# dalek-cryptography/curve25519-dalek

Measured on NVIDIA H100. Metric: Pippenger MSM points/sec, higher is better.
Workload: dtype exact integers: f64 limbs (radix 2^51, FP64 pipe) in the bucket kernel, u32 limbs (radix 2^25.5) elsewhere

## Files before the change

### curve25519_dalek_b200/csrc/engine.h

```cpp
#pragma once
#include <cuda_runtime.h>
#include <stddef.h>
#include <stdint.h>
#include <cstdio>
#include <string>
#include <utility>
#include <vector>

#include "../../include/dalek_b200.h"
#include "ge.cuh"

struct DevBuf {
    void *p = nullptr;
    size_t cap = 0;
};

struct dalek_b200_ctx {
    int device = 0;
    int sm_count = 132;
    cudaStream_t stream = nullptr;
    cudaStream_t stream2 = nullptr;
    cudaStream_t stream_copy = nullptr;
    cudaStream_t stream3 = nullptr;
    cudaStream_t stream_hash = nullptr;
    cudaEvent_t ev_hram[8] = {};
    cudaEvent_t ev_a = nullptr, ev_b = nullptr, ev_fork = nullptr, ev_join = nullptr, ev_join2 = nullptr;
    cudaEvent_t ev_call0 = nullptr, ev_call1 = nullptr;
    cudaEvent_t ev_prep[8][2] = {};
    int prep_pieces = 0;
    float last_prep_ms = 0.f;
    cudaEvent_t ev_grp[8] = {nullptr, nullptr, nullptr, nullptr, nullptr, nullptr, nullptr, nullptr};
    std::string last_error;
    uint64_t launches = 0;
    long opt_window_bits = 0;
    long opt_verify_chunk = 0;
    long opt_host_chunks = 8;
    long opt_trace = 0;
    long opt_precomp_tables = 0;
    long opt_double_base_comb = 1;
    long opt_dedupe_keys = 1;
    long opt_verify_pieces = 4;
    long opt_decompress_f64 = 1;
    long opt_acc_tma = 0;
    long opt_transcript_warp = 1;
    long opt_transcript_blocks = 1;
    long opt_each_comb = 1;
    long opt_small_straus = 1;
    long opt_field_f64 = 1;
    float last_kernel_ms = 0.f;
    float last_call_ms = 0.f;
    int last_kernel_launches = 0;
    bool async_open = false;
    DevBuf scalars, points_in, points, digits, counts, offsets, sorted, buckets, red_a, red_b, red_c,
        red_d, key_pts, result, flags, misc0, misc1, misc2, misc3, misc4, misc5, zs, base_table, ntasks, task_off, tasks, task_sums, msg_offs, sum_desc, sum_part, key_table, key_acc, task_order, sig_status, misc6, each_pow, each_tab, each_kstat;
    DevBuf prep_prod;
    uint32_t hash_seed[4] = {0x243F6A88u, 0x85A308D3u, 0x13198A2Eu, 0x03707344u};
    int sum_desc_c = -1;
    bool base_table_ready = false;
    bool each_attr_set = false;
    bool comb_attr_set = false;
    DevBuf comb_base_table;
    bool comb_base_table_ready = false;
    void *h_pinned = nullptr;
    size_t h_pinned_cap = 0;
    size_t last_zs_n = 0;
    std::vector<std::pair<const char *, cudaEvent_t>> trace;
};

#define CUDA_TRY(ctx, expr)                                                                      \
    do {                                                                                         \
        cudaError_t _e = (expr);                                                                 \
        if (_e != cudaSuccess) {                                                                 \
            (ctx)->last_error = std::string(#expr) + ": " + cudaGetErrorString(_e);              \
            return -3;                                                                           \
        }                                                                                        \
    } while (0)

inline float elapsed_ms(cudaEvent_t a, cudaEvent_t b)
{
    float ms = 0.f;
    if (cudaEventElapsedTime(&ms, a, b) == cudaSuccess) return ms;
    cudaGetLastError();
    return -1.f;
}

struct CallTimer {
    dalek_b200_ctx *ctx;
    explicit CallTimer(dalek_b200_ctx *c) : ctx(c) { if (ctx) cudaEventRecord(ctx->ev_call0, ctx->stream); }
    ~CallTimer()
    {
        if (!ctx) return;
        float ms = 0.f;
        if (cudaEventRecord(ctx->ev_call1, ctx->stream) == cudaSuccess && cudaEventSynchronize(ctx->ev_call1) == cudaSuccess &&
            (ms = elapsed_ms(ctx->ev_call0, ctx->ev_call1)) >= 0.f)
            ctx->last_call_ms = ms;
    }
};

inline void trace_mark(dalek_b200_ctx *ctx, const char *name, cudaStream_t st)
{
    if (!ctx->opt_trace) return;
    cudaEvent_t e;
    if (cudaEventCreate(&e) != cudaSuccess) return;
    cudaEventRecord(e, st);
    ctx->trace.push_back({name, e});
}
inline void trace_dump(dalek_b200_ctx *ctx)
{
    if (!ctx->opt_trace) return;
    cudaDeviceSynchronize();
// ... 66 lines not shown
```

### curve25519_dalek_b200/csrc/msm.cu

```cuda
#include <algorithm>
#include <cstdio>
#include <utility>
#include <vector>

#include "../../include/dalek_b200.h"
#include "engine.h"
#include "ge64.cuh"
#include "warp4.cuh"
#include "warp4_f64.cuh"

static inline unsigned cdiv(size_t a, unsigned b) { return (unsigned)((a + b - 1) / b); }

int ws_reserve(dalek_b200_ctx *ctx, DevBuf &b, size_t bytes)
{
    if (bytes <= b.cap) return 0;
    if (b.p) { cudaFree(b.p); b.p = nullptr; b.cap = 0; }
    size_t want = bytes + bytes / 8 + 256;
    cudaError_t e = cudaMalloc(&b.p, want);
    if (e != cudaSuccess) { ctx->last_error = std::string("cudaMalloc: ") + cudaGetErrorString(e); return DALEK_E_NOMEM; }
    b.cap = want;
    return 0;
}

int pinned_reserve(dalek_b200_ctx *ctx, size_t bytes)
{
    if (bytes <= ctx->h_pinned_cap) return 0;
    if (ctx->h_pinned) cudaFreeHost(ctx->h_pinned);
    ctx->h_pinned = nullptr; ctx->h_pinned_cap = 0;
    cudaError_t e = cudaMallocHost(&ctx->h_pinned, bytes + 4096);
    if (e != cudaSuccess) { ctx->last_error = std::string("cudaMallocHost: ") + cudaGetErrorString(e); return DALEK_E_NOMEM; }
    ctx->h_pinned_cap = bytes + 4096;
    return 0;
}

template <int F64>
__global__ void __launch_bounds__(128, 3) k_prep_compressed(const uint4 *__restrict__ in, ge_niels_packed *__restrict__ out, size_t n,
                                  int *__restrict__ bad)
{
    size_t i = (size_t)blockIdx.x * blockDim.x + threadIdx.x;
    if (i >= n) return;
    uint4 a = in[2 * i], b = in[2 * i + 1];
    uint32_t s[8] = {a.x, a.y, a.z, a.w, b.x, b.y, b.z, b.w};
    fe x, y;
    uint32_t ok = ge_decompress_affine<F64>(x, y, s);
    if (!ok) { atomicOr(bad, 1); fe_0(x); fe_1(y); }
    ge_niels nl; ge_affine_to_niels(nl, x, y);
    ge_niels_packed p; ge_niels_pack(p, nl);
    uint4 *o = reinterpret_cast<uint4 *>(out + i);
#pragma unroll
    for (int k = 0; k < 6; k++) o[k] = make_uint4(p.w[4 * k], p.w[4 * k + 1], p.w[4 * k + 2], p.w[4 * k + 3]);
}

template <int F64>
__global__ void k_prep_ristretto(const uint32_t *__restrict__ in, ge_niels_packed *__restrict__ out, size_t n, int *__restrict__ bad)
{
    size_t i = (size_t)blockIdx.x * blockDim.x + threadIdx.x;
    if (i >= n) return;
    uint32_t enc[8];
#pragma unroll
    for (int k = 0; k < 8; k++) enc[k] = in[8 * i + k];
    ge_p3 P;
// ... 756 lines not shown
                }
            }
        };
        if (len) prefetch(e_next, 0);
        if (!TMA) asm volatile("cp.async.commit_group;" ::: "memory");
        for (uint32_t k = 0; k < len; k++) {
            const uint32_t e = e_next, neg = e >> 31;
            const int buf = k & 1;
            if (k + 1 < len) { e_next = idx[k + 1]; prefetch(e_next, buf ^ 1); }
            uint32_t words[NQ * 4];
            if (TMA) {
                const uint32_t bar = (uint32_t)__cvta_generic_to_shared(&s_bar[buf][threadIdx.x]);
                const uint32_t parity = (k >> 1) & 1u;
                uint32_t done;
                do {
                    asm volatile("{ .reg .pred p; mbarrier.try_wait.parity.shared::cta.b64 p, [%1], %2; selp.u32 %0, 1, 0, p; }"
                                 : "=r"(done) : "r"(bar), "r"(parity) : "memory");
                } while (!done);
                const uint4 *sp = reinterpret_cast<const uint4 *>(&s_bulk[buf][threadIdx.x][0]);
#pragma unroll
                for (int q = 0; q < NQ; q++) { uint4 v = sp[q]; words[4 * q] = v.x; words[4 * q + 1] = v.y; words[4 * q + 2] = v.z; words[4 * q + 3] = v.w; }
            } else {
                asm volatile("cp.async.commit_group;" ::: "memory");
                asm volatile("cp.async.wait_group 1;" ::: "memory");
#pragma unroll
                for (int q = 0; q < NQ; q++) { uint4 v = s_pts[buf][q][threadIdx.x]; words[4 * q] = v.x; words[4 * q + 1] = v.y; words[4 * q + 2] = v.z; words[4 * q + 3] = v.w; }
            }
            ge_niels_packed pk;
#pragma unroll
            for (int q = 0; q < 24; q++) pk.w[q] = words[q];
            ge64_niels nl; ge64_niels_unpack(nl, pk);
            ge64_madd(acc64, acc64, nl, neg);
        }
        ge64_to_p3(acc, acc64);
    } else {
    if (fold_old) load_p3(acc, buckets + t); else ge_p3_identity(acc);
    for (uint32_t k = 0; k < len; k++) {
        uint32_t e = idx[k];
        uint32_t neg = e >> 31, pi = e & 0x7fffffffu;
        const uint4 *src = reinterpret_cast<const uint4 *>(reinterpret_cast<const ge_niels_packed *>(points) + pi);
        ge_niels_packed pk;
#pragma unroll
        for (int q = 0; q < 6; q++) { uint4 v = __ldg(src + q); pk.w[4 * q] = v.x; pk.w[4 * q + 1] = v.y; pk.w[4 * q + 2] = v.z; pk.w[4 * q + 3] = v.w; }
        ge_niels nl; ge_niels_unpack(nl, pk);
        ge_madd(acc, acc, nl, neg);
    }
    }
    ge_p3_raw r; ge_p3_store_raw(r, acc);
    uint4 *o = reinterpret_cast<uint4 *>(!split ? buckets + t : task_sums + p);
#pragma unroll
    for (int q = 0; q < 10; q++) o[q] = make_uint4(r.w[4 * q], r.w[4 * q + 1], r.w[4 * q + 2], r.w[4 * q + 3]);
}


__global__ void __launch_bounds__(128)
k_heavy_fixup(const uint32_t *__restrict__ heavy, const uint32_t *__restrict__ ntasks, const uint32_t *__restrict__ task_off,
              const uint32_t *__restrict__ win_base, uint32_t nbuckets, uint32_t w0, uint32_t w1,
              const ge_p3_raw *__restrict__ task_sums, ge_p3_raw *__restrict__ buckets, int first)
{
    const uint32_t lane = threadIdx.x & 31, role = lane & 3, grp = lane >> 2;
    const uint32_t nwarps = (gridDim.x * blockDim.x) >> 5;
    const uint32_t nheavy = heavy[0];
    for (uint32_t h = (blockIdx.x * blockDim.x + threadIdx.x) >> 5; h < nheavy; h += nwarps) {
        uint32_t tb = heavy[1 + h];
        if (tb / nbuckets < w0 || tb / nbuckets >= w1) continue;
        uint32_t kk = ntasks[tb];
        uint32_t base = win_base[tb / nbuckets] + task_off[tb];
        w4_point acc, x;
        if (first || grp != 0) w4_identity(acc); else w4_load(acc, buckets + tb);
        for (uint32_t j0 = 0; j0 < kk; j0 += 8) {
            uint32_t j = j0 + grp;
            if (j < kk) w4_load(x, task_sums + base + j); else w4_identity(x);
            w4_add(acc, x, role);
        }
        for (int d = 16; d >= 4; d >>= 1) { w4_shfl_down(x, acc, d); w4_add(acc, x, role); }
        if (grp == 0) w4_store(buckets + tb, acc, role);
    }
}

__device__ __forceinline__ void load_p3_f64(ge64_p3 &o, const ge_p3_raw *src)
{
    ge_p3 q; load_p3(q, src);
    fe64_from_fe_limbs(o.X, q.X); fe64_from_fe_limbs(o.Y, q.Y); fe64_from_fe_limbs(o.Z, q.Z); fe64_from_fe_limbs(o.T, q.T);
}

__global__ void __launch_bounds__(32)
k_chunk_reduce_f64(const ge_p3_raw *__restrict__ S_in, uint32_t n_in, uint32_t m, uint32_t n_out, uint32_t nwin,
                   ge_p3_raw *__restrict__ S_out, ge_p3_raw *__restrict__ W_out)
{
    const uint32_t t = blockIdx.x * blockDim.x + threadIdx.x;
    if (t >= n_out * nwin) return;
    const uint32_t w = t / n_out, q = t % n_out;
    const ge_p3_raw *S = S_in + (size_t)w * n_in + (size_t)q * m;
    fe64 d2; fe64_const_2d(d2);
    ge64_p3 run, acc, x;
    load_p3_f64(run, S + (m - 1));
    acc = run;
    ge_p3 nxt;
    if (m > 1) load_p3(nxt, S + (m - 2));
#pragma unroll 1
    for (uint32_t r = m - 1; r-- > 0;) {
        fe64_from_fe_limbs(x.X, nxt.X); fe64_from_fe_limbs(x.Y, nxt.Y); fe64_from_fe_limbs(x.Z, nxt.Z); fe64_from_fe_limbs(x.T, nxt.T);
        if (r > 0) load_p3(nxt, S + (r - 1));
        ge64_add_p3(run, run, x, d2);
        ge64_add_p3(acc, acc, run, d2);
    }
    ge_p3 o; ge_p3_raw raw;
    ge64_to_p3(o, run); ge_p3_store_raw(raw, o);
    uint4 *d = reinterpret_cast<uint4 *>(S_out + t);
#pragma unroll
    for (int k = 0; k < 10; k++) d[k] = make_uint4(raw.w[4 * k], raw.w[4 * k + 1], raw.w[4 * k + 2], raw.w[4 * k + 3]);
    ge64_to_p3(o, acc); ge_p3_store_raw(raw, o);
    d = reinterpret_cast<uint4 *>(W_out + t);
#pragma unroll
    for (int k = 0; k < 10; k++) d[k] = make_uint4(raw.w[4 * k], raw.w[4 * k + 1], raw.w[4 * k + 2], raw.w[4 * k + 3]);
}

__global__ void __launch_bounds__(128)
k_chunk_reduce(const ge_p3_raw *__restrict__ S_in, uint32_t n_in, uint32_t m, uint32_t one_based, uint32_t n_out,
               uint32_t nwin, ge_p3_raw *__restrict__ S_out, ge_p3_raw *__restrict__ W_out)
{
    const uint32_t role = threadIdx.x & 3;
    const uint32_t total = n_out * nwin;
    uint32_t t = (blockIdx.x * blockDim.x + threadIdx.x) >> 2;
    if (((blockIdx.x * blockDim.x + (threadIdx.x & ~31u)) >> 2) >= total) return;
    const bool live = t < total;
    if (!live) t = total - 1;
    const uint32_t w = t / n_out, q = t % n_out;
    const ge_p3_raw *S = S_in + (size_t)w * n_in + (size_t)q * m;
    w4_point run, acc, x;
    w4_load(run, S + (m - 1));
    acc = run;
    for (uint32_t r = m - 1; r-- > 1;) {
        w4_load(x, S + r);
        w4_add(run, x, role);
        w4_add(acc, run, role);
    }
    if (m > 1) {
        w4_load(x, S);
        w4_add(run, x, role);
        if (one_based) w4_add(acc, run, role);
    } else if (!one_based) {
        w4_identity(acc);
    }
    if (live) { w4_store(S_out + t, run, role); w4_store(W_out + t, acc, role); }
}

#define SUM_PIECE 256u
__global__ void __launch_bounds__(128)
k_plain_sum(const ge_p3_raw *__restrict__ pool, const uint2 *__restrict__ desc, ge_p3_raw *__restrict__ out)
{
    __shared__ ge_p3_raw sh[32];
    const uint32_t role = threadIdx.x & 3, grp = threadIdx.x >> 2;
    const uint2 d = desc[blockIdx.x];
    const ge_p3_raw *a = pool + d.x;
    const uint32_t len = d.y;
    w4_point acc, x;
    w4_identity(acc);
    for (uint32_t i0 = 0; i0 < len; i0 += 32) {
        uint32_t i = i0 + grp;
        if (i < len) w4_load(x, a + i); else w4_identity(x);
        w4_add(acc, x, role);
    }
    w4_store(&sh[grp], acc, role);
    __syncthreads();
    for (uint32_t d = 16; d > 0; d >>= 1) {
        if (threadIdx.x < 32 * ((d + 7) / 8)) {
            uint32_t g2 = grp < d ? grp + d : grp;
            w4_load(acc, &sh[grp]); w4_load(x, &sh[g2]);
            w4_add(acc, x, role);
        }
        __syncthreads();
        if (grp < d) w4_store(&sh[grp], acc, role);
        __syncthreads();
    }
    if (grp == 0) { w4_load(acc, &sh[0]); w4_store(out + blockIdx.x, acc, role); }
}

struct LevelInfo { int nlevels; int log2m[16]; };
__global__ void __launch_bounds__(128)
k_finish_windows(const ge_p3_raw *__restrict__ S_top, const ge_p3_raw *__restrict__ A, LevelInfo li, uint32_t nwin,
                 ge_p3_raw *__restrict__ out)
{
    const uint32_t role = threadIdx.x & 3;
    uint32_t w = (blockIdx.x * blockDim.x + threadIdx.x) >> 2;
    if (((blockIdx.x * blockDim.x + (threadIdx.x & ~31u)) >> 2) >= nwin) return;
    const bool live = w < nwin;
    if (!live) w = nwin - 1;
    w4_point t, x;
    if (li.nlevels > 0) {
        w4_load(t, A + (size_t)(li.nlevels - 1) * nwin + w);
        for (int l = li.nlevels - 2; l >= 0; l--) {
            for (int k = 0; k < li.log2m[l]; k++) w4_dbl(t, role, k == li.log2m[l] - 1);
            w4_load(x, A + (size_t)l * nwin + w);
            w4_add(t, x, role);
        }
    } else {
        w4_load(t, S_top + w);
    }
    if (live) w4_store(out + w, t, role);
}

__global__ void __launch_bounds__(32)
k_combine(const ge_p3_raw *__restrict__ windows, int ranks, int nwin, int c, MsmResult *__restrict__ res)
{
    const uint32_t role = threadIdx.x & 3;
    w4f_point tot;
    w4f_horner(tot, windows, ranks, nwin, c, role);
    if (threadIdx.x != 0) return;
    ge_p3 total; w4f_to_p3(total, tot);
    uint32_t s[8];
    ge_compress(s, total);
#pragma unroll
    for (int i = 0; i < 8; i++) res->compressed[i] = s[i];
    fe_to_limbs51(res->limbs, total.X); fe_to_limbs51(res->limbs + 5, total.Y);
    fe_to_limbs51(res->limbs + 10, total.Z); fe_to_limbs51(res->limbs + 15, total.T);
    res->is_identity = ge_is_identity(total);
    res->pad = 0;
}

static int msm_sort_fine_bits(size_t entries_per_window, int c, int hist_windows)
{
    int lg = std::max(0, c - 1 - SORT_FINE_MAX);
    while (lg < c - 1 && ((size_t)SORT_BIN_MEAN << lg) < entries_per_window && (2u << lg) <= SORT_NC_MAX &&
           ((size_t)hist_windows << (lg + 1)) <= SORT_HIST_MAX)
        lg++;
    return c - 1 - lg;
}

int msm_accumulate_chunk(dalek_b200_ctx *ctx, const uint32_t *d_scalars, const ge_niels_packed *d_points, size_t n,
                         int c, bool first, int active_windows, size_t flat, cudaEvent_t points_ready)
{
    const int nwin_d = msm_window_count_for_bits(c);
    const int nact = active_windows > 0 && active_windows < nwin_d ? active_windows : nwin_d;
    const int nwin = flat ? 1 : nwin_d;
    const uint32_t nb = 1u << (c - 1);
    const size_t total_buckets = (size_t)nwin * nb;
    const uint32_t task_len = flat ? msm_task_len(n * (size_t)nact, 1, nb) : msm_task_len(n, nact, nb);
    const size_t max_tasks = total_buckets + (std::max<size_t>(1, n) * nact) / task_len + 1;
    const size_t max_heavy = (std::max<size_t>(1, n) * nact) / task_len + 1;
    const uint32_t parts = (nb + SCAN_PART - 1) / SCAN_PART;
    const int F = msm_sort_fine_bits(flat ? n * (size_t)nact : n, c, flat ? 1 : nact);
    const uint32_t nc = nb >> F;
    cudaStream_t st = ctx->stream;
    int rc;
    if ((rc = ws_reserve(ctx, ctx->counts, (total_buckets + (size_t)nwin * nc + 1 + max_heavy) * 4))) return rc;
    if ((rc = ws_reserve(ctx, ctx->offsets, (total_buckets + (size_t)nwin * parts + 2 * (size_t)nwin * nc + nwin) * 4))) return rc;
    if ((rc = ws_reserve(ctx, ctx->ntasks, total_buckets * 4))) return rc;
    if ((rc = ws_reserve(ctx, ctx->task_off, total_buckets * 4 + (nwin + 1) * 4))) return rc;
    if ((rc = ws_reserve(ctx, ctx->tasks, max_tasks * 8))) return rc;
    if ((rc = ws_reserve(ctx, ctx->task_sums, max_tasks * sizeof(ge_p3_raw)))) return rc;
    if ((rc = ws_reserve(ctx, ctx->task_order, (3 * TASK_BINS + max_tasks) * 4))) return rc;
    if ((rc = ws_reserve(ctx, ctx->digits, std::max<size_t>(1, n) * nact * 8))) return rc;
    if ((rc = ws_reserve(ctx, ctx->sorted, std::max<size_t>(1, n) * nact * 4))) return rc;
    if ((rc = ws_reserve(ctx, ctx->buckets, total_buckets * sizeof(ge_p3_raw)))) return rc;
    uint32_t *counts = (uint32_t *)ctx->counts.p, *offsets = (uint32_t *)ctx->offsets.p;
    uint32_t *ntasks = (uint32_t *)ctx->ntasks.p, *task_off = (uint32_t *)ctx->task_off.p;
    uint32_t *win_base = task_off + total_buckets;
    uint32_t *ccount = counts + total_buckets, *heavy = ccount + (size_t)nwin * nc;
    uint32_t *part_sums = offsets + total_buckets, *ccursor = part_sums + (size_t)nwin * parts;
    uint32_t *xpre = ccursor + (size_t)nwin * nc, *xtot = xpre + (size_t)nwin * nc;
    uint2 *tasks = (uint2 *)ctx->tasks.p;
    uint32_t *t_hist = (uint32_t *)ctx->task_order.p, *t_cursor = t_hist + TASK_BINS, *t_start = t_cursor + TASK_BINS;
    uint32_t *order = t_start + TASK_BINS;
    ge_p3_raw *task_sums = (ge_p3_raw *)ctx->task_sums.p;
    uint2 *records = (uint2 *)ctx->digits.p;
    uint32_t *sorted = (uint32_t *)ctx->sorted.p;
    ge_p3_raw *buckets = (ge_p3_raw *)ctx->buckets.p;

    const size_t part_smem = SORT_TILE * 8 + (2 * (size_t)nc + 33) * 4;
    const size_t fine_smem = SORT_FINE_CAP * 12 + ((1u << F) + 33) * 4;
    CUDA_TRY(ctx, cudaFuncSetAttribute(k_sort_partition, cudaFuncAttributeMaxDynamicSharedMemorySize, (int)part_smem));
    CUDA_TRY(ctx, cudaFuncSetAttribute(k_sort_fine, cudaFuncAttributeMaxDynamicSharedMemorySize, (int)fine_smem));
    CUDA_TRY(ctx, cudaMemsetAsync(ccount, 0, ((size_t)nwin * nc + 1) * 4, st));
    CUDA_TRY(ctx, cudaMemsetAsync(t_hist, 0, 2 * TASK_BINS * 4, st));
    if (n) {
        k_sort_count<<<cdiv(n, SORT_COUNT_TILE), SORT_THREADS, 0, st>>>((const uint4 *)d_scalars, n, c, nact, F, nc, flat ? 1 : 0, ccount);
        ctx->launches++;
    }
    k_sort_bins_scan<<<nwin, SORT_THREADS, 0, st>>>(ccount, nc, F, nb, ccursor, xpre, xtot, counts, ntasks);
    if (n) {
        k_sort_partition<<<cdiv(n, SORT_TILE), SORT_THREADS, part_smem, st>>>((const uint4 *)d_scalars, n, c, nact, F, nc, nb, flat,
                                                                              ccount, ccursor, records, counts);
        ctx->launches++;
    }
    const size_t extra = n * (size_t)nact / SORT_FINE_CAP;
    k_sort_fine<<<(unsigned)(nwin * nc + extra), SORT_THREADS, fine_smem, st>>>(records, ccount, ccursor, xpre, xtot, n, F, nc, nb,
                                                                               (uint32_t)nwin, flat ? 1 : 0, counts, offsets, sorted, ntasks);
    k_task_count<<<cdiv(total_buckets, 256), 256, 0, st>>>(counts, (uint32_t)total_buckets, task_len, ntasks, heavy);
    k_scan_partial<<<nwin * parts, 1024, 0, st>>>(ntasks, nb, parts, part_sums);
    k_scan_bases<<<nwin, 32, 0, st>>>(part_sums, parts);
    k_scan_apply<<<nwin * parts, 1024, 0, st>>>(ntasks, part_sums, nb, parts, task_off);
    k_task_bases<<<1, 32, 0, st>>>(ntasks, task_off, nb, nwin, win_base);
    k_task_fill<<<cdiv(total_buckets, 256), 256, 0, st>>>(ntasks, task_off, win_base, nb, (uint32_t)total_buckets, tasks);
    k_task_hist<<<cdiv(max_tasks, 256), 256, 0, st>>>(tasks, counts, win_base + nwin, task_len, t_hist);
    k_task_scan<<<1, 256, 0, st>>>(t_hist, t_start);
    k_task_scatter<<<cdiv(max_tasks, 256), 256, 0, st>>>(tasks, counts, win_base + nwin, task_len, t_start, t_cursor, order);
    ctx->launches += 11;
    if (points_ready) CUDA_TRY(ctx, cudaStreamWaitEvent(st, points_ready, 0));
    if (first) CUDA_TRY(ctx, cudaEventRecord(ctx->ev_a, st));
    {
        const unsigned grid = cdiv(max_tasks, 128);
        const int f = first ? 1 : 0;
#define LAUNCH_ACC(F64_, TMA_) k_bucket_accumulate<F64_, TMA_><<<grid, 128, 0, st>>>(d_points, sorted, counts, offsets, ntasks, tasks, order, win_base, 0, nwin, n, nb, task_len, buckets, task_sums, f)
        const bool tma = ctx->opt_field_f64 && ctx->opt_acc_tma;
        if (tma) LAUNCH_ACC(1, 1); else if (ctx->opt_field_f64) LAUNCH_ACC(1, 0); else LAUNCH_ACC(0, 0);
#undef LAUNCH_ACC
        k_heavy_fixup<<<ctx->sm_count * 4, 128, 0, st>>>(heavy, ntasks, task_off, win_base, nb, 0u, (uint32_t)nwin, task_sums, buckets, f);
        ctx->launches += 2;
    }
    CUDA_TRY(ctx, cudaEventRecord(ctx->ev_b, st));
    ctx->last_kernel_launches = first ? 1 : ctx->last_kernel_launches + 1;
    CUDA_TRY(ctx, cudaGetLastError());
    return 0;
}

int msm_reduce_finish(dalek_b200_ctx *ctx, int c, ge_p3_raw *d_windows, MsmResult *d_result, bool flat)
{
    const int nwin = flat ? 1 : msm_window_count_for_bits(c);
    const int desc_key = c + (flat ? 64 : 0);
    const uint32_t nb = 1u << (c - 1);
    cudaStream_t st = ctx->stream;
    int rc;
    ge_p3_raw *buckets = (ge_p3_raw *)ctx->buckets.p;
    LevelInfo li; li.nlevels = 0;
    std::vector<uint32_t> lvl_m, lvl_nout;
    size_t pool_pts = 0;
    {
        uint32_t n_in = nb; bool first = true;
        while (n_in > 1) {
            uint32_t m = first ? std::min<uint32_t>(n_in, 16) : std::min<uint32_t>(n_in, 8);
            uint32_t n_out = (n_in + m - 1) / m;
            lvl_m.push_back(m); lvl_nout.push_back(n_out);
            int lg = 0; while ((1u << lg) < m) lg++;
            li.log2m[li.nlevels++] = lg;
            pool_pts += 2 * (size_t)n_out * nwin;
            n_in = n_out; first = false;
        }
    }
    if ((rc = ws_reserve(ctx, ctx->red_a, std::max<size_t>(1, pool_pts) * sizeof(ge_p3_raw)))) return rc;
    if ((rc = ws_reserve(ctx, ctx->red_b, (size_t)16 * nwin * sizeof(ge_p3_raw)))) return rc;
    ge_p3_raw *pool = (ge_p3_raw *)ctx->red_a.p, *A = (ge_p3_raw *)ctx->red_b.p;
    const ge_p3_raw *S_in = buckets;
    uint32_t n_in = nb;
    size_t pos = 0;
    std::vector<std::pair<size_t, uint32_t>> w_arrays;
    for (int l = 0; l < li.nlevels; l++) {
        uint32_t m = lvl_m[l], n_out = lvl_nout[l];
        ge_p3_raw *S_out = pool + pos, *W_out = pool + pos + (size_t)n_out * nwin;
        if (l == 0 && ctx->opt_field_f64 && n_in % m == 0)
            k_chunk_reduce_f64<<<cdiv((size_t)n_out * nwin, 32), 32, 0, st>>>(S_in, n_in, m, n_out, nwin, S_out, W_out);
        else
            k_chunk_reduce<<<cdiv((size_t)n_out * nwin * 4, 128), 128, 0, st>>>(S_in, n_in, m, l == 0 ? 1u : 0u, n_out, nwin, S_out, W_out);
        ctx->launches++;
        w_arrays.push_back({pos + (size_t)n_out * nwin, n_out});
        S_in = S_out; n_in = n_out; pos += 2 * (size_t)n_out * nwin;
    }
    {
        std::vector<uint2> d1, d2;
        for (int l = 0; l < li.nlevels; l++)
            for (int w = 0; w < nwin; w++) {
                uint32_t off = (uint32_t)(w_arrays[l].first + (size_t)w * w_arrays[l].second), len = w_arrays[l].second;
                uint32_t first_piece = (uint32_t)d1.size();
                for (uint32_t o = 0; o < len; o += SUM_PIECE) d1.push_back(make_uint2(off + o, std::min(SUM_PIECE, len - o)));
                d2.push_back(make_uint2(first_piece, (uint32_t)d1.size() - first_piece));
            }
        const size_t n1 = d1.size(), n2 = d2.size();
        if ((rc = ws_reserve(ctx, ctx->sum_desc, (n1 + n2) * sizeof(uint2)))) return rc;
        if ((rc = ws_reserve(ctx, ctx->sum_part, n1 * sizeof(ge_p3_raw)))) return rc;
        uint2 *dd1 = (uint2 *)ctx->sum_desc.p, *dd2 = dd1 + n1;
        if (ctx->sum_desc_c != desc_key) {
            CUDA_TRY(ctx, cudaMemcpyAsync(dd1, d1.data(), n1 * sizeof(uint2), cudaMemcpyHostToDevice, st));
            CUDA_TRY(ctx, cudaMemcpyAsync(dd2, d2.data(), n2 * sizeof(uint2), cudaMemcpyHostToDevice, st));
            CUDA_TRY(ctx, cudaStreamSynchronize(st));
            ctx->sum_desc_c = desc_key;
        }
        ge_p3_raw *parts = (ge_p3_raw *)ctx->sum_part.p;
        k_plain_sum<<<(unsigned)n1, 128, 0, st>>>(pool, dd1, parts);
        k_plain_sum<<<(unsigned)n2, 128, 0, st>>>(parts, dd2, A);
        ctx->launches += 2;
    }
    k_finish_windows<<<cdiv((size_t)nwin * 4, 128), 128, 0, st>>>(S_in, A, li, nwin, d_windows);
    ctx->launches++;
    if (d_result) {
        k_combine<<<1, 32, 0, st>>>(d_windows, 1, nwin, c, d_result);
        ctx->launches++;
    }
    CUDA_TRY(ctx, cudaGetLastError());
    return 0;
}

int msm_combine_windows(dalek_b200_ctx *ctx, const ge_p3_raw *d_windows, int ranks, int nwin, int c, MsmResult *d_result)
{
    k_combine<<<1, 32, 0, ctx->stream>>>(d_windows, ranks, nwin, c, d_result);
    ctx->launches++;
    CUDA_TRY(ctx, cudaGetLastError());
    return 0;
}
```

### curve25519_dalek_b200/csrc/warp4.cuh

```cuda
#pragma once
#include "ge.cuh"

struct w4_point { fe X, Y, Z, T; };

__device__ __forceinline__ void fe_sel4(fe &o, const fe &a0, const fe &a1, const fe &a2, const fe &a3, uint32_t role)
{
    const uint32_t m0 = 0u - (uint32_t)(role == 0), m1 = 0u - (uint32_t)(role == 1);
    const uint32_t m2 = 0u - (uint32_t)(role == 2), m3 = 0u - (uint32_t)(role == 3);
#pragma unroll
    for (int i = 0; i < 10; i++) o.v[i] = (a0.v[i] & m0) | (a1.v[i] & m1) | (a2.v[i] & m2) | (a3.v[i] & m3);
}

__device__ __forceinline__ void fe_gbcast(fe &o, const fe &mine, int i)
{
    const int src = (int)((threadIdx.x & 28u) | (uint32_t)i);
#pragma unroll
    for (int k = 0; k < 10; k++) o.v[k] = __shfl_sync(0xffffffffu, mine.v[k], src);
}

__device__ __forceinline__ void w4_identity(w4_point &p) { fe_0(p.X); fe_1(p.Y); fe_1(p.Z); fe_0(p.T); }

__device__ __forceinline__ void w4_load(w4_point &p, const ge_p3_raw *src)
{
    const uint4 *s = reinterpret_cast<const uint4 *>(src);
    ge_p3_raw r;
#pragma unroll
    for (int q = 0; q < 10; q++) { uint4 v = s[q]; r.w[4 * q] = v.x; r.w[4 * q + 1] = v.y; r.w[4 * q + 2] = v.z; r.w[4 * q + 3] = v.w; }
#pragma unroll
    for (int i = 0; i < 10; i++) { p.X.v[i] = r.w[i]; p.Y.v[i] = r.w[10 + i]; p.Z.v[i] = r.w[20 + i]; p.T.v[i] = r.w[30 + i]; }
}

__device__ __forceinline__ void w4_store(ge_p3_raw *dst, const w4_point &p, uint32_t role)
{
    fe mine; fe_sel4(mine, p.X, p.Y, p.Z, p.T, role);
    uint32_t *o = dst->w + 10 * role;
#pragma unroll
    for (int i = 0; i < 10; i += 2) *reinterpret_cast<uint2 *>(o + i) = make_uint2(mine.v[i], mine.v[i + 1]);
}

__device__ __forceinline__ void w4_dbl(w4_point &p, uint32_t role, bool want_t)
{
    fe S, in, r, XX, YY, ZZ, S2, t, Xc, Yc, Zc, Tc, f, g;
    fe_add(S, p.X, p.Y);
    fe_sel4(in, p.X, p.Y, p.Z, S, role);
    fe_sq(r, in);
    fe_gbcast(XX, r, 0); fe_gbcast(YY, r, 1); fe_gbcast(ZZ, r, 2); fe_gbcast(S2, r, 3);
    fe_sub(t, S2, YY); fe_sub(t, t, XX); fe_carry(Xc, t);
    fe_add(Yc, YY, XX);
    fe_sub(Zc, YY, XX);
    fe_add(t, ZZ, ZZ); fe_add(t, t, XX); fe_sub(Tc, t, YY);
    fe_sel4(f, Tc, Zc, Tc, Yc, role);
    fe_sel4(g, Xc, Yc, Zc, Xc, role);
    fe_mul(r, f, g);
    fe_gbcast(p.X, r, 0); fe_gbcast(p.Y, r, 1); fe_gbcast(p.Z, r, 2);
    if (want_t) fe_gbcast(p.T, r, 3);
}

__device__ __forceinline__ void w4_add(w4_point &p, const w4_point &q, uint32_t role)
{
    fe d2, qYpX, qYmX, qT2d, A, B, f, g, r, a, b, c, zz, D, E, H, DpC, DmC, t;
    fe_const_2d(d2);
    fe_add(t, q.Y, q.X); fe_carry(qYpX, t);
    fe_sub(t, q.Y, q.X); fe_carry(qYmX, t);
    fe_sub(A, p.Y, p.X); fe_add(B, p.Y, p.X);
    fe_mul(qT2d, q.T, d2);
    fe_sel4(f, A, B, p.T, p.Z, role);
    fe_sel4(g, qYmX, qYpX, qT2d, q.Z, role);
    fe_mul(r, f, g);
    fe_gbcast(a, r, 0); fe_gbcast(b, r, 1); fe_gbcast(c, r, 2); fe_gbcast(zz, r, 3);
    fe_add(D, zz, zz);
    fe_sub(E, b, a); fe_add(H, b, a); fe_add(DpC, D, c); fe_sub(DmC, D, c);
    fe_sel4(f, DmC, DpC, DmC, E, role);
    fe_sel4(g, E, H, DpC, H, role);
    fe_mul(r, f, g);
    fe_gbcast(p.X, r, 0); fe_gbcast(p.Y, r, 1); fe_gbcast(p.Z, r, 2); fe_gbcast(p.T, r, 3);
}

__device__ __forceinline__ void w4_shfl_down(w4_point &o, const w4_point &p, int delta_lanes)
{
#pragma unroll
    for (int i = 0; i < 10; i++) {
        o.X.v[i] = __shfl_down_sync(0xffffffffu, p.X.v[i], delta_lanes);
        o.Y.v[i] = __shfl_down_sync(0xffffffffu, p.Y.v[i], delta_lanes);
        o.Z.v[i] = __shfl_down_sync(0xffffffffu, p.Z.v[i], delta_lanes);
        o.T.v[i] = __shfl_down_sync(0xffffffffu, p.T.v[i], delta_lanes);
    }
}
```

### curve25519_dalek_b200/csrc/warp4_f64.cuh

```cuda
#pragma once
#include "ge64.cuh"

#if defined(__CUDACC__)
#define W4_DEV __device__ __forceinline__
W4_DEV uint32_t w4_lane() { return threadIdx.x & 31u; }
W4_DEV uint32_t w4_shfl(uint32_t v, int src) { return __shfl_sync(0xffffffffu, v, src); }
W4_DEV uint32_t w4_shfl_down(uint32_t v, int delta) { return __shfl_down_sync(0xffffffffu, v, delta); }
W4_DEV bool w4_any(bool p) { return __any_sync(0xffffffffu, p) != 0; }
W4_DEV long long w4_bits(double d) { return __double_as_longlong(d); }
W4_DEV double w4_from_bits(long long b) { return __longlong_as_double(b); }
#else
#include <string.h>
#define W4_DEV static inline
uint32_t w4_lane();
uint32_t w4_shfl(uint32_t v, int src);
uint32_t w4_shfl_down(uint32_t v, int delta);
bool w4_any(bool p);
W4_DEV long long w4_bits(double d) { long long b; memcpy(&b, &d, 8); return b; }
W4_DEV double w4_from_bits(long long b) { double d; memcpy(&d, &b, 8); return d; }
#endif

struct w4f_point { fe64 X, Y, Z, T; };

W4_DEV void fe64_sel4(fe64 &o, const fe64 &a0, const fe64 &a1, const fe64 &a2, const fe64 &a3, uint32_t role)
// ... 204 lines not shown
    const long long limb = rr + qp;
#if FE64_DEV
    return __longlong_as_double((limb + (1LL << 51)) | FE64_E52) - (FE64_TWO52 + FE64_TWO51);
#else
    assert(limb < (1LL << 50) + (1LL << 15) && limb > -(1LL << 50) - (1LL << 15));
    return (double)limb;
#endif
}

W4_DEV double w20_take(const w4f_point &p, const w20_role &r)
{
    double v = 0.0;
#pragma unroll
    for (uint32_t k = 0; k < 5; k++) {
        const double x = r.g == 0 ? p.X.v[k] : r.g == 1 ? p.Y.v[k] : r.g == 2 ? p.Z.v[k] : p.T.v[k];
        if (r.i == k) v = x;
    }
    return v;
}
W4_DEV void w20_give(w4f_point &p, double c)
{
#pragma unroll
    for (uint32_t k = 0; k < 5; k++) {
        p.X.v[k] = w20_shfl(c, k); p.Y.v[k] = w20_shfl(c, 5u + k); p.Z.v[k] = w20_shfl(c, 10u + k); p.T.v[k] = w20_shfl(c, 15u + k);
    }
}

W4_DEV void w20_dbl(double &c, const w20_role &r)
{
    const double x = w20_shfl(c, r.i), y = w20_shfl(c, 5u + r.i);
    const double s = w20_carry(x + y, r);
    const double in = r.g == 3 ? s : c;
    const double sq = w20_mul(in, in, r);
    const double xx = w20_shfl(sq, r.i), yy = w20_shfl(sq, 5u + r.i), zz = w20_shfl(sq, 10u + r.i), s2 = w20_shfl(sq, 15u + r.i);
    const double Yp = yy + xx, Ym = yy - xx;
    const double E = s2 - Yp;
    const double F = w20_carry(zz + zz - Ym, r);
    const double a = r.g == 1 ? Yp : r.g == 2 ? Ym : E;
    const double b = r.g == 1 ? Ym : r.g == 3 ? Yp : F;
    c = w20_mul(a, b, r);
}

W4_DEV void w20_dbl_n(w4f_point &p, int k)
{
    const w20_role r = w20_roles();
    double c = w20_take(p, r);
#if FE64_DEV
#pragma unroll 1
#endif
    for (int t = 0; t < k; t++) w20_dbl(c, r);
    w20_give(p, c);
}

W4_DEV void w4f_horner(w4f_point &tot, const ge_p3_raw *windows, int ranks, int nwin, int c, uint32_t role)
{
    fe64 d2; fe64_const_2d(d2);
    w4f_point x;
    w4f_identity(tot);
    bool started = false;
#pragma unroll 1
    for (int w = nwin - 1; w >= 0; w--) {
        if (started) {
            w20_dbl_n(tot, c);
        } else {
            bool any = false;
#pragma unroll 1
            for (int r = 0; r < ranks; r++) {
                ge_p3 q; ge_p3_raw raw;
#if defined(__CUDA_ARCH__)
                const uint4 *s4 = reinterpret_cast<const uint4 *>(windows + (size_t)r * nwin + w);
#pragma unroll
                for (int k = 0; k < 10; k++) { uint4 v = s4[k]; raw.w[4 * k] = v.x; raw.w[4 * k + 1] = v.y; raw.w[4 * k + 2] = v.z; raw.w[4 * k + 3] = v.w; }
#else
                raw = windows[(size_t)r * nwin + w];
#endif
                ge_p3_load_raw(q, raw);
                any |= !ge_is_identity(q);
            }
            if (!any) continue;
            started = true;
        }
#pragma unroll 1
        for (int r = 0; r < ranks; r++) { w4f_load(x, windows + (size_t)r * nwin + w); w4f_add(tot, x, d2, role); }
    }
}
```

Measured before the change: 362.5 million.

## Port reduction kernels to f64 warp arithmetic, add persistent chunk reduce and empty-skip

Rewrites heavy-bucket fixup to use per-thread f64 adds for small task counts and warp-level f64 reduction for large ones. Chunk reduce at level 0 becomes a persistent atomic-scheduled kernel that skips empty bucket ranges using counts when only one accumulation chunk ran. Remaining warp4 u32 kernels (higher levels, sums, horner combine) switch to the f64 w4f variants, and final compression uses a distributed 20-lane inversion. The intent is moving reduction work to the FP64 pipe and cutting idle work on empty buckets, at the cost of an extra memset and an occupancy query.

```diff
diff --git a/curve25519_dalek_b200/csrc/engine.h b/curve25519_dalek_b200/csrc/engine.h
--- a/curve25519_dalek_b200/csrc/engine.h
+++ b/curve25519_dalek_b200/csrc/engine.h
@@ -56,6 +56,8 @@
     DevBuf prep_prod;
     uint32_t hash_seed[4] = {0x243F6A88u, 0x85A308D3u, 0x13198A2Eu, 0x03707344u};
     int sum_desc_c = -1;
+    int acc_chunks = 0;
+    int reduce_warps = 0;
     bool base_table_ready = false;
     bool each_attr_set = false;
     bool comb_attr_set = false;
diff --git a/curve25519_dalek_b200/csrc/msm.cu b/curve25519_dalek_b200/csrc/msm.cu
--- a/curve25519_dalek_b200/csrc/msm.cu
+++ b/curve25519_dalek_b200/csrc/msm.cu
@@ -6,7 +6,6 @@
 #include "../../include/dalek_b200.h"
 #include "engine.h"
 #include "ge64.cuh"
-#include "warp4.cuh"
 #include "warp4_f64.cuh"
 
 static inline unsigned cdiv(size_t a, unsigned b) { return (unsigned)((a + b - 1) / b); }
@@ -869,73 +868,117 @@
     for (int q = 0; q < 10; q++) o[q] = make_uint4(r.w[4 * q], r.w[4 * q + 1], r.w[4 * q + 2], r.w[4 * q + 3]);
 }
 
-
+__device__ __forceinline__ void load_p3_f64(ge64_p3 &o, const ge_p3_raw *src)
+{
+    ge_p3 q; load_p3(q, src);
+    fe64_from_fe_limbs(o.X, q.X); fe64_from_fe_limbs(o.Y, q.Y); fe64_from_fe_limbs(o.Z, q.Z); fe64_from_fe_limbs(o.T, q.T);
+}
+
+__device__ __forceinline__ void store_p3_f64(ge_p3_raw *dst, const ge64_p3 &p)
+{
+    ge_p3 o; ge_p3_raw raw;
+    ge64_to_p3(o, p); ge_p3_store_raw(raw, o);
+    uint4 *d = reinterpret_cast<uint4 *>(dst);
+#pragma unroll
+    for (int k = 0; k < 10; k++) d[k] = make_uint4(raw.w[4 * k], raw.w[4 * k + 1], raw.w[4 * k + 2], raw.w[4 * k + 3]);
+}
+
+#define HEAVY_LANE_MAX 16u
 __global__ void __launch_bounds__(128)
 k_heavy_fixup(const uint32_t *__restrict__ heavy, const uint32_t *__restrict__ ntasks, const uint32_t *__restrict__ task_off,
               const uint32_t *__restrict__ win_base, uint32_t nbuckets, uint32_t w0, uint32_t w1,
               const ge_p3_raw *__restrict__ task_sums, ge_p3_raw *__restrict__ buckets, int first)
 {
-    const uint32_t lane = threadIdx.x & 31, role = lane & 3, grp = lane >> 2;
-    const uint32_t nwarps = (gridDim.x * blockDim.x) >> 5;
+    const uint32_t nthreads = gridDim.x * blockDim.x, nwarps = nthreads >> 5, lane = threadIdx.x & 31;
     const uint32_t nheavy = heavy[0];
+    fe64 d2; fe64_const_2d(d2);
+    for (uint32_t h = blockIdx.x * blockDim.x + threadIdx.x; h < nheavy; h += nthreads) {
+        const uint32_t tb = heavy[1 + h], kk = ntasks[tb];
+        if (tb / nbuckets < w0 || tb / nbuckets >= w1 || kk > HEAVY_LANE_MAX) continue;
+        const uint32_t base = win_base[tb / nbuckets] + task_off[tb];
+        ge64_p3 acc, x;
+        uint32_t j = 0;
+        if (first) { load_p3_f64(acc, task_sums + base); j = 1; } else load_p3_f64(acc, buckets + tb);
+#pragma unroll 1
+        for (; j < kk; j++) { load_p3_f64(x, task_sums + base + j); ge64_add_p3(acc, acc, x, d2); }
+        store_p3_f64(buckets + tb, acc);
+    }
     for (uint32_t h = (blockIdx.x * blockDim.x + threadIdx.x) >> 5; h < nheavy; h += nwarps) {
-        uint32_t tb = heavy[1 + h];
-        if (tb / nbuckets < w0 || tb / nbuckets >= w1) continue;
-        uint32_t kk = ntasks[tb];
-        uint32_t base = win_base[tb / nbuckets] + task_off[tb];
-        w4_point acc, x;
-        if (first || grp != 0) w4_identity(acc); else w4_load(acc, buckets + tb);
-        for (uint32_t j0 = 0; j0 < kk; j0 += 8) {
-            uint32_t j = j0 + grp;
-            if (j < kk) w4_load(x, task_sums + base + j); else w4_identity(x);
-            w4_add(acc, x, role);
-        }
-        for (int d = 16; d >= 4; d >>= 1) { w4_shfl_down(x, acc, d); w4_add(acc, x, role); }
-        if (grp == 0) w4_store(buckets + tb, acc, role);
-    }
-}
-
-__device__ __forceinline__ void load_p3_f64(ge64_p3 &o, const ge_p3_raw *src)
-{
-    ge_p3 q; load_p3(q, src);
-    fe64_from_fe_limbs(o.X, q.X); fe64_from_fe_limbs(o.Y, q.Y); fe64_from_fe_limbs(o.Z, q.Z); fe64_from_fe_limbs(o.T, q.T);
+        const uint32_t tb = heavy[1 + h], kk = ntasks[tb];
+        if (tb / nbuckets < w0 || tb / nbuckets >= w1 || kk <= HEAVY_LANE_MAX) continue;
+        const uint32_t base = win_base[tb / nbuckets] + task_off[tb];
+        ge64_p3 acc, x;
+        if (first || lane != 0) ge64_identity(acc); else load_p3_f64(acc, buckets + tb);
+#pragma unroll 1
+        for (uint32_t j = lane; j < kk; j += 32) { load_p3_f64(x, task_sums + base + j); ge64_add_p3(acc, acc, x, d2); }
+        for (int d = 16; d > 0; d >>= 1) {
+            fe64_shfl_down(x.X, acc.X, d); fe64_shfl_down(x.Y, acc.Y, d); fe64_shfl_down(x.Z, acc.Z, d); fe64_shfl_down(x.T, acc.T, d);
+            ge64_add_p3(acc, acc, x, d2);
+        }
+        if (lane == 0) store_p3_f64(buckets + tb, acc);
+    }
 }
 
 __global__ void __launch_bounds__(32)
 k_chunk_reduce_f64(const ge_p3_raw *__restrict__ S_in, uint32_t n_in, uint32_t m, uint32_t n_out, uint32_t nwin,
+                   const uint32_t *__restrict__ counts, uint32_t *__restrict__ next, ge_p3_raw *__restrict__ S_out,
+                   ge_p3_raw *__restrict__ W_out)
+{
+    const uint32_t total = n_out * nwin, lane = threadIdx.x & 31;
+    fe64 d2; fe64_const_2d(d2);
+#pragma unroll 1
+    for (;;) {
+        uint32_t base = 0;
+        if (lane == 0) base = atomicAdd(next, 32u);
+        base = __shfl_sync(0xffffffffu, base, 0);
+        if (base >= total) return;
+        const uint32_t t = base + lane;
+        if (t < total) {
+            const uint32_t w = t / n_out, q = t % n_out;
+            const size_t b0 = (size_t)w * n_in + (size_t)q * m;
+            bool empty = counts != nullptr;
+            if (counts) {
+#pragma unroll 1
+                for (uint32_t r = 0; r < m; r += 4) {
+                    const uint4 v = *reinterpret_cast<const uint4 *>(counts + b0 + r);
+                    empty &= (v.x | v.y | v.z | v.w) == 0;
+                }
+            }
+            ge64_p3 run, acc, x;
+            if (empty) {
+                ge64_identity(run); acc = run;
+            } else {
+                const ge_p3_raw *S = S_in + b0;
+                load_p3_f64(run, S + (m - 1));
+                acc = run;
+                ge_p3 nxt;
+                if (m > 1) load_p3(nxt, S + (m - 2));
+#pragma unroll 1
+                for (uint32_t r = m - 1; r-- > 0;) {
+                    fe64_from_fe_limbs(x.X, nxt.X); fe64_from_fe_limbs(x.Y, nxt.Y); fe64_from_fe_limbs(x.Z, nxt.Z); fe64_from_fe_limbs(x.T, nxt.T);
+                    if (r > 0) load_p3(nxt, S + (r - 1));
+                    ge64_add_p3(run, run, x, d2);
+                    ge64_add_p3(acc, acc, run, d2);
+                }
+            }
+            store_p3_f64(S_out + t, run);
+            store_p3_f64(W_out + t, acc);
+        }
+    }
+}
+
+__device__ __forceinline__ void w4f_store(ge_p3_raw *dst, const w4f_point &p, uint32_t role)
+{
+    fe64 mine; fe64_sel4(mine, p.X, p.Y, p.Z, p.T, role);
+    fe f; fe64_to_fe(f, mine);
+    uint32_t *o = dst->w + 10 * role;
+#pragma unroll
+    for (int i = 0; i < 10; i += 2) *reinterpret_cast<uint2 *>(o + i) = make_uint2(f.v[i], f.v[i + 1]);
+}
+
+__global__ void __launch_bounds__(128)
+k_chunk_reduce_w4f(const ge_p3_raw *__restrict__ S_in, uint32_t n_in, uint32_t m, uint32_t n_out, uint32_t nwin,
                    ge_p3_raw *__restrict__ S_out, ge_p3_raw *__restrict__ W_out)
-{
-    const uint32_t t = blockIdx.x * blockDim.x + threadIdx.x;
-    if (t >= n_out * nwin) return;
-    const uint32_t w = t / n_out, q = t % n_out;
-    const ge_p3_raw *S = S_in + (size_t)w * n_in + (size_t)q * m;
-    fe64 d2; fe64_const_2d(d2);
-    ge64_p3 run, acc, x;
-    load_p3_f64(run, S + (m - 1));
-    acc = run;
-    ge_p3 nxt;
-    if (m > 1) load_p3(nxt, S + (m - 2));
-#pragma unroll 1
-    for (uint32_t r = m - 1; r-- > 0;) {
-        fe64_from_fe_limbs(x.X, nxt.X); fe64_from_fe_limbs(x.Y, nxt.Y); fe64_from_fe_limbs(x.Z, nxt.Z); fe64_from_fe_limbs(x.T, nxt.T);
-        if (r > 0) load_p3(nxt, S + (r - 1));
-        ge64_add_p3(run, run, x, d2);
-        ge64_add_p3(acc, acc, run, d2);
-    }
-    ge_p3 o; ge_p3_raw raw;
-    ge64_to_p3(o, run); ge_p3_store_raw(raw, o);
-    uint4 *d = reinterpret_cast<uint4 *>(S_out + t);
-#pragma unroll
-    for (int k = 0; k < 10; k++) d[k] = make_uint4(raw.w[4 * k], raw.w[4 * k + 1], raw.w[4 * k + 2], raw.w[4 * k + 3]);
-    ge64_to_p3(o, acc); ge_p3_store_raw(raw, o);
-    d = reinterpret_cast<uint4 *>(W_out + t);
-#pragma unroll
-    for (int k = 0; k < 10; k++) d[k] = make_uint4(raw.w[4 * k], raw.w[4 * k + 1], raw.w[4 * k + 2], raw.w[4 * k + 3]);
-}
-
-__global__ void __launch_bounds__(128)
-k_chunk_reduce(const ge_p3_raw *__restrict__ S_in, uint32_t n_in, uint32_t m, uint32_t one_based, uint32_t n_out,
-               uint32_t nwin, ge_p3_raw *__restrict__ S_out, ge_p3_raw *__restrict__ W_out)
 {
     const uint32_t role = threadIdx.x & 3;
     const uint32_t total = n_out * nwin;
@@ -945,22 +988,19 @@
     if (!live) t = total - 1;
     const uint32_t w = t / n_out, q = t % n_out;
     const ge_p3_raw *S = S_in + (size_t)w * n_in + (size_t)q * m;
-    w4_point run, acc, x;
-    w4_load(run, S + (m - 1));
+    fe64 d2; fe64_const_2d(d2);
+    w4f_point run, acc, x;
+    w4f_load(run, S + (m - 1));
     acc = run;
+#pragma unroll 1
     for (uint32_t r = m - 1; r-- > 1;) {
-        w4_load(x, S + r);
-        w4_add(run, x, role);
-        w4_add(acc, run, role);
-    }
-    if (m > 1) {
-        w4_load(x, S);
-        w4_add(run, x, role);
-        if (one_based) w4_add(acc, run, role);
-    } else if (!one_based) {
-        w4_identity(acc);
-    }
-    if (live) { w4_store(S_out + t, run, role); w4_store(W_out + t, acc, role); }
+        w4f_load(x, S + r);
+        w4f_add(run, x, d2, role);
+        w4f_add(acc, run, d2, role);
+    }
+    if (m > 1) { w4f_load(x, S); w4f_add(run, x, d2, role); }
+    else w4f_identity(acc);
+    if (live) { w4f_store(S_out + t, run, role); w4f_store(W_out + t, acc, role); }
 }
 
 #define SUM_PIECE 256u
@@ -972,26 +1012,27 @@
     const uint2 d = desc[blockIdx.x];
     const ge_p3_raw *a = pool + d.x;
     const uint32_t len = d.y;
-    w4_point acc, x;
-    w4_identity(acc);
+    fe64 d2; fe64_const_2d(d2);
+    w4f_point acc, x;
+    w4f_identity(acc);
     for (uint32_t i0 = 0; i0 < len; i0 += 32) {
         uint32_t i = i0 + grp;
-        if (i < len) w4_load(x, a + i); else w4_identity(x);
-        w4_add(acc, x, role);
-    }
-    w4_store(&sh[grp], acc, role);
+        if (i < len) w4f_load(x, a + i); else w4f_identity(x);
+        w4f_add(acc, x, d2, role);
+    }
+    w4f_store(&sh[grp], acc, role);
     __syncthreads();
     for (uint32_t d = 16; d > 0; d >>= 1) {
         if (threadIdx.x < 32 * ((d + 7) / 8)) {
             uint32_t g2 = grp < d ? grp + d : grp;
-            w4_load(acc, &sh[grp]); w4_load(x, &sh[g2]);
-            w4_add(acc, x, role);
+            w4f_load(acc, &sh[grp]); w4f_load(x, &sh[g2]);
+            w4f_add(acc, x, d2, role);
         }
         __syncthreads();
-        if (grp < d) w4_store(&sh[grp], acc, role);
+        if (grp < d) w4f_store(&sh[grp], acc, role);
         __syncthreads();
     }
-    if (grp == 0) { w4_load(acc, &sh[0]); w4_store(out + blockIdx.x, acc, role); }
+    if (grp == 0) { w4f_load(acc, &sh[0]); w4f_store(out + blockIdx.x, acc, role); }
 }
 
 struct LevelInfo { int nlevels; int log2m[16]; };
@@ -1004,18 +1045,19 @@
     if (((blockIdx.x * blockDim.x + (threadIdx.x & ~31u)) >> 2) >= nwin) return;
     const bool live = w < nwin;
     if (!live) w = nwin - 1;
-    w4_point t, x;
+    fe64 d2; fe64_const_2d(d2);
+    w4f_point t, x;
     if (li.nlevels > 0) {
-        w4_load(t, A + (size_t)(li.nlevels - 1) * nwin + w);
+        w4f_load(t, A + (size_t)(li.nlevels - 1) * nwin + w);
         for (int l = li.nlevels - 2; l >= 0; l--) {
-            for (int k = 0; k < li.log2m[l]; k++) w4_dbl(t, role, k == li.log2m[l] - 1);
-            w4_load(x, A + (size_t)l * nwin + w);
-            w4_add(t, x, role);
+            for (int k = 0; k < li.log2m[l]; k++) w4f_dbl(t, role, k == li.log2m[l] - 1);
+            w4f_load(x, A + (size_t)l * nwin + w);
+            w4f_add(t, x, d2, role);
         }
     } else {
-        w4_load(t, S_top + w);
-    }
-    if (live) w4_store(out + w, t, role);
+        w4f_load(t, S_top + w);
+    }
+    if (live) w4f_store(out + w, t, role);
 }
 
 __global__ void __launch_bounds__(32)
@@ -1024,10 +1066,10 @@
     const uint32_t role = threadIdx.x & 3;
     w4f_point tot;
     w4f_horner(tot, windows, ranks, nwin, c, role);
+    uint32_t s[8];
+    w20_compress(s, tot);
     if (threadIdx.x != 0) return;
     ge_p3 total; w4f_to_p3(total, tot);
-    uint32_t s[8];
-    ge_compress(s, total);
 #pragma unroll
     for (int i = 0; i < 8; i++) res->compressed[i] = s[i];
     fe_to_limbs51(res->limbs, total.X); fe_to_limbs51(res->limbs + 5, total.Y);
@@ -1128,6 +1170,7 @@
     }
     CUDA_TRY(ctx, cudaEventRecord(ctx->ev_b, st));
     ctx->last_kernel_launches = first ? 1 : ctx->last_kernel_launches + 1;
+    ctx->acc_chunks = first ? 1 : ctx->acc_chunks + 1;
     CUDA_TRY(ctx, cudaGetLastError());
     return 0;
 }
@@ -1156,8 +1199,15 @@
         }
     }
     if ((rc = ws_reserve(ctx, ctx->red_a, std::max<size_t>(1, pool_pts) * sizeof(ge_p3_raw)))) return rc;
-    if ((rc = ws_reserve(ctx, ctx->red_b, (size_t)16 * nwin * sizeof(ge_p3_raw)))) return rc;
+    if ((rc = ws_reserve(ctx, ctx->red_b, (size_t)16 * nwin * sizeof(ge_p3_raw) + 4))) return rc;
     ge_p3_raw *pool = (ge_p3_raw *)ctx->red_a.p, *A = (ge_p3_raw *)ctx->red_b.p;
+    uint32_t *next = (uint32_t *)(A + (size_t)16 * nwin);
+    if (!ctx->reduce_warps) {
+        int per_sm = 0;
+        CUDA_TRY(ctx, cudaOccupancyMaxActiveBlocksPerMultiprocessor(&per_sm, k_chunk_reduce_f64, 32, 0));
+        ctx->reduce_warps = std::max(1, per_sm) * ctx->sm_count;
+    }
+    CUDA_TRY(ctx, cudaMemsetAsync(next, 0, 4, st));
     const ge_p3_raw *S_in = buckets;
     uint32_t n_in = nb;
     size_t pos = 0;
@@ -1165,10 +1215,13 @@
     for (int l = 0; l < li.nlevels; l++) {
         uint32_t m = lvl_m[l], n_out = lvl_nout[l];
         ge_p3_raw *S_out = pool + pos, *W_out = pool + pos + (size_t)n_out * nwin;
-        if (l == 0 && ctx->opt_field_f64 && n_in % m == 0)
-            k_chunk_reduce_f64<<<cdiv((size_t)n_out * nwin, 32), 32, 0, st>>>(S_in, n_in, m, n_out, nwin, S_out, W_out);
-        else
-            k_chunk_reduce<<<cdiv((size_t)n_out * nwin * 4, 128), 128, 0, st>>>(S_in, n_in, m, l == 0 ? 1u : 0u, n_out, nwin, S_out, W_out);
+        if (l == 0) {
+            const unsigned grid = std::min<unsigned>(cdiv((size_t)n_out * nwin, 32), (unsigned)ctx->reduce_warps);
+            const uint32_t *cnt = ctx->acc_chunks == 1 ? (const uint32_t *)ctx->counts.p : nullptr;
+            k_chunk_reduce_f64<<<grid, 32, 0, st>>>(S_in, n_in, m, n_out, nwin, cnt, next, S_out, W_out);
+        } else {
+            k_chunk_reduce_w4f<<<cdiv((size_t)n_out * nwin * 4, 128), 128, 0, st>>>(S_in, n_in, m, n_out, nwin, S_out, W_out);
+        }
         ctx->launches++;
         w_arrays.push_back({pos + (size_t)n_out * nwin, n_out});
         S_in = S_out; n_in = n_out; pos += 2 * (size_t)n_out * nwin;
diff --git a/curve25519_dalek_b200/csrc/warp4.cuh b/curve25519_dalek_b200/csrc/warp4.cuh
--- a/curve25519_dalek_b200/csrc/warp4.cuh
+++ b/curve25519_dalek_b200/csrc/warp4.cuh
@@ -1,7 +1,5 @@
 #pragma once
 #include "ge.cuh"
-
-struct w4_point { fe X, Y, Z, T; };
 
 __device__ __forceinline__ void fe_sel4(fe &o, const fe &a0, const fe &a1, const fe &a2, const fe &a3, uint32_t role)
 {
@@ -10,79 +8,3 @@
 #pragma unroll
     for (int i = 0; i < 10; i++) o.v[i] = (a0.v[i] & m0) | (a1.v[i] & m1) | (a2.v[i] & m2) | (a3.v[i] & m3);
 }
-
-__device__ __forceinline__ void fe_gbcast(fe &o, const fe &mine, int i)
-{
-    const int src = (int)((threadIdx.x & 28u) | (uint32_t)i);
-#pragma unroll
-    for (int k = 0; k < 10; k++) o.v[k] = __shfl_sync(0xffffffffu, mine.v[k], src);
-}
-
-__device__ __forceinline__ void w4_identity(w4_point &p) { fe_0(p.X); fe_1(p.Y); fe_1(p.Z); fe_0(p.T); }
-
-__device__ __forceinline__ void w4_load(w4_point &p, const ge_p3_raw *src)
-{
-    const uint4 *s = reinterpret_cast<const uint4 *>(src);
-    ge_p3_raw r;
-#pragma unroll
-    for (int q = 0; q < 10; q++) { uint4 v = s[q]; r.w[4 * q] = v.x; r.w[4 * q + 1] = v.y; r.w[4 * q + 2] = v.z; r.w[4 * q + 3] = v.w; }
-#pragma unroll
-    for (int i = 0; i < 10; i++) { p.X.v[i] = r.w[i]; p.Y.v[i] = r.w[10 + i]; p.Z.v[i] = r.w[20 + i]; p.T.v[i] = r.w[30 + i]; }
-}
-
-__device__ __forceinline__ void w4_store(ge_p3_raw *dst, const w4_point &p, uint32_t role)
-{
-    fe mine; fe_sel4(mine, p.X, p.Y, p.Z, p.T, role);
-    uint32_t *o = dst->w + 10 * role;
-#pragma unroll
-    for (int i = 0; i < 10; i += 2) *reinterpret_cast<uint2 *>(o + i) = make_uint2(mine.v[i], mine.v[i + 1]);
-}
-
-__device__ __forceinline__ void w4_dbl(w4_point &p, uint32_t role, bool want_t)
-{
-    fe S, in, r, XX, YY, ZZ, S2, t, Xc, Yc, Zc, Tc, f, g;
-    fe_add(S, p.X, p.Y);
-    fe_sel4(in, p.X, p.Y, p.Z, S, role);
-    fe_sq(r, in);
-    fe_gbcast(XX, r, 0); fe_gbcast(YY, r, 1); fe_gbcast(ZZ, r, 2); fe_gbcast(S2, r, 3);
-    fe_sub(t, S2, YY); fe_sub(t, t, XX); fe_carry(Xc, t);
-    fe_add(Yc, YY, XX);
-    fe_sub(Zc, YY, XX);
-    fe_add(t, ZZ, ZZ); fe_add(t, t, XX); fe_sub(Tc, t, YY);
-    fe_sel4(f, Tc, Zc, Tc, Yc, role);
-    fe_sel4(g, Xc, Yc, Zc, Xc, role);
-    fe_mul(r, f, g);
-    fe_gbcast(p.X, r, 0); fe_gbcast(p.Y, r, 1); fe_gbcast(p.Z, r, 2);
-    if (want_t) fe_gbcast(p.T, r, 3);
-}
-
-__device__ __forceinline__ void w4_add(w4_point &p, const w4_point &q, uint32_t role)
-{
-    fe d2, qYpX, qYmX, qT2d, A, B, f, g, r, a, b, c, zz, D, E, H, DpC, DmC, t;
-    fe_const_2d(d2);
-    fe_add(t, q.Y, q.X); fe_carry(qYpX, t);
-    fe_sub(t, q.Y, q.X); fe_carry(qYmX, t);
-    fe_sub(A, p.Y, p.X); fe_add(B, p.Y, p.X);
-    fe_mul(qT2d, q.T, d2);
-    fe_sel4(f, A, B, p.T, p.Z, role);
-    fe_sel4(g, qYmX, qYpX, qT2d, q.Z, role);
-    fe_mul(r, f, g);
-    fe_gbcast(a, r, 0); fe_gbcast(b, r, 1); fe_gbcast(c, r, 2); fe_gbcast(zz, r, 3);
-    fe_add(D, zz, zz);
-    fe_sub(E, b, a); fe_add(H, b, a); fe_add(DpC, D, c); fe_sub(DmC, D, c);
-    fe_sel4(f, DmC, DpC, DmC, E, role);
-    fe_sel4(g, E, H, DpC, H, role);
-    fe_mul(r, f, g);
-    fe_gbcast(p.X, r, 0); fe_gbcast(p.Y, r, 1); fe_gbcast(p.Z, r, 2); fe_gbcast(p.T, r, 3);
-}
-
-__device__ __forceinline__ void w4_shfl_down(w4_point &o, const w4_point &p, int delta_lanes)
-{
-#pragma unroll
-    for (int i = 0; i < 10; i++) {
-        o.X.v[i] = __shfl_down_sync(0xffffffffu, p.X.v[i], delta_lanes);
-        o.Y.v[i] = __shfl_down_sync(0xffffffffu, p.Y.v[i], delta_lanes);
-        o.Z.v[i] = __shfl_down_sync(0xffffffffu, p.Z.v[i], delta_lanes);
-        o.T.v[i] = __shfl_down_sync(0xffffffffu, p.T.v[i], delta_lanes);
-    }
-}
diff --git a/curve25519_dalek_b200/csrc/warp4_f64.cuh b/curve25519_dalek_b200/csrc/warp4_f64.cuh
--- a/curve25519_dalek_b200/csrc/warp4_f64.cuh
+++ b/curve25519_dalek_b200/csrc/warp4_f64.cuh
@@ -280,6 +280,51 @@
     w20_give(p, c);
 }
 
+W4_DEV double w20_own(const fe64 &f, const w20_role &r)
+{
+    double v = 0.0;
+#pragma unroll
+    for (uint32_t k = 0; k < 5; k++) if (r.i == k) v = f.v[k];
+    return v;
+}
+W4_DEV double w20_sqn(double a, int n, const w20_role &r)
+{
+#if FE64_DEV
+#pragma unroll 1
+#endif
+    for (int k = 0; k < n; k++) a = w20_mul(a, a, r);
+    return a;
+}
+W4_DEV double w20_invert(double z, const w20_role &r)
+{
+    const double t0 = w20_mul(z, z, r);
+    const double t2 = w20_mul(z, w20_sqn(t0, 2, r), r);
+    const double t3 = w20_mul(t0, t2, r);
+    const double t5 = w20_mul(t2, w20_mul(t3, t3, r), r);
+    const double t7 = w20_mul(w20_sqn(t5, 5, r), t5, r);
+    const double t9 = w20_mul(w20_sqn(t7, 10, r), t7, r);
+    const double t11 = w20_mul(w20_sqn(t9, 20, r), t9, r);
+    const double t13 = w20_mul(w20_sqn(t11, 10, r), t7, r);
+    const double t15 = w20_mul(w20_sqn(t13, 50, r), t13, r);
+    const double t17 = w20_mul(w20_sqn(t15, 100, r), t15, r);
+    const double t19 = w20_mul(w20_sqn(t17, 50, r), t13, r);
+    return w20_mul(w20_sqn(t19, 5, r), t3, r);
+}
+
+W4_DEV void w20_compress(uint32_t s[8], const w4f_point &p)
+{
+    const w20_role r = w20_roles();
+    const double zi = w20_invert(w20_own(p.Z, r), r);
+    const double xy = w20_mul(w20_take(p, r), zi, r);
+    fe64 x, y;
+#pragma unroll
+    for (uint32_t k = 0; k < 5; k++) { x.v[k] = w20_shfl(xy, k); y.v[k] = w20_shfl(xy, 5u + k); }
+    fe fx, fy;
+    fe64_to_fe(fx, x); fe64_to_fe(fy, y);
+    fe_tobytes_words(s, fy);
+    s[7] ^= (uint32_t)fe_isnegative(fx) << 31;
+}
+
 W4_DEV void w4f_horner(w4f_point &tot, const ge_p3_raw *windows, int ranks, int nwin, int c, uint32_t role)
 {
     fe64 d2; fe64_const_2d(d2);
```

New measurement: 375.0 million (median of 6 runs). 1.03x the previous value.
